# lssfau/ExaStencils

Measured on AMD Instinct MI355X. Metric: LU/s, higher is better.
Workload: dtype f64; 1 GPU; 3D Poisson 7-point Jacobi smoother steps (ghost exchange + sweep + advance), 512 x 512 x 512 cells per GPU, reference field layout (515-double rows); three consecutive steps per pass over HBM (temporal blocking, bit-identical); levels=9, align=0

## Files before the change

### exastencils_amd/csrc/kernels_twostage.hip

```cpp
#include "examg_common.h"

#include <type_traits>

namespace examg {

struct TSGeom {
  int ntx, nty, ntz, zc, nblocks, remap;
  int xs;
  int ys, zs;
  int first;
  Box box1;
  int ax0, ax1, ay0, ay1, az0, az1;
};

constexpr int TS_OUT = 124;

__device__ __forceinline__ long long uniform64(long long v) {
  const unsigned lo = __builtin_amdgcn_readfirstlane((unsigned)v), hi = __builtin_amdgcn_readfirstlane((unsigned)((unsigned long long)v >> 32));
  return (long long)(((unsigned long long)hi << 32) | lo);
}

struct TSProl {
  LayoutDev lc;
  const double *uc;
// ... 498 lines not shown
#undef EXAMG_TS_LAUNCH_ORD
#undef EXAMG_TS_LAUNCH_PF
#undef EXAMG_TS_LAUNCH
  EXAMG_CHECK_LAUNCH("k_two_stage7_lds");
  return 0;
}

template <bool COL>
static int launch_two_stage(const examg_layout_t *lu_, const double *u, const examg_layout_t *lf_, const double *rhs,
                            double *out, const examg_stencil_t *st, double w, int first, const Box &box, hipStream_t s,
                            const Box *box1 = nullptr, const TSProl *prol = nullptr, bool zero_in = false) {
  const Box &b1 = box1 ? *box1 : box;
  int impl = g_ts_lds == -2 ? (box.n1() >= 192 ? 8 : 5) : g_ts_lds;
  if (zero_in && impl == 6) impl = 5;
  if (g_ts_lds == -2 && impl == 8 && !prol && !zero_in && box.count() >= 50000000LL) impl = 83;
  if (impl == 83 && !prol && !zero_in)
    return launch_two_stage_lds<COL, 8, 1, 3>(lu_, u, lf_, rhs, out, st, w, first, box, b1, s, prol, zero_in);
  if (impl == 83) impl = 8;
  if (impl == 8) return launch_two_stage_lds<COL, 8>(lu_, u, lf_, rhs, out, st, w, first, box, b1, s, prol, zero_in);
  if (impl == 6) return launch_two_stage_lds<COL, 6>(lu_, u, lf_, rhs, out, st, w, first, box, b1, s, prol, zero_in);
  return launch_two_stage_lds<COL, 5>(lu_, u, lf_, rhs, out, st, w, first, box, b1, s, prol, zero_in);
}

static bool prolong_args_ok(const char *who, const examg_layout_t *lc, const Box &box) {
  if (box.b0 < 0 || box.b1 < 0 || box.b2 < 0) { set_error("%s: negative fine index", who); return false; }
  int32_t cb[3] = {box.b0 / 2, box.b1 / 2, box.b2 / 2}, ce[3] = {box.e0 / 2 + 1, box.e1 / 2 + 1, box.e2 / 2 + 1};
  if (lc->nd != 3 || !box_inside(lc, make_box(cb, ce), 0)) { set_error("%s: coarse footprint leaves the coarse allocation", who); return false; }
  return true;
}

static bool two_stage_ok(const examg_layout_t *lu, const examg_layout_t *lf, const examg_stencil_t *st, const Box &box) {
  return !g_ts_disable && !lay_split(lu) && !lay_split(lf) && lu->nd == 3 && canonical_order7(st) >= 0 && box.n0() >= 64 && box_inside(lu, box, 1) &&
         box_inside(lf, box, 0);
}

static bool stage_boxes_ok(const examg_layout_t *lf_, const Box &box1, const Box &box2) {
  const LayoutDev lf = make_layout(lf_);
  const bool lo = box1.b0 < box2.b0 && box2.b1 + lf.ref1 == 0 && box2.b2 + lf.ref2 == 0;
  const bool hi = box1.e0 > box2.e0 && box2.e1 + lf.ref1 == lf.tot1 && box2.e2 + lf.ref2 == lf.tot2;
  return !lo && !hi;
}

constexpr int TS3_OUT = 120;

template <int ORDER, int NW, bool NT, int RPW = 3, bool COL = false>
__global__ void __launch_bounds__(64 * NW, 1)
k_three_stage7_lds(LayoutDev lu, const double *__restrict__ u, LayoutDev lf, const double *__restrict__ rhs,
                   double *__restrict__ out, Coef7 k, double w, Box box, TSGeom g) {
  constexpr int NS = RPW * NW;
  constexpr int NO = NS - 4;
  __shared__ d2 SM[3 * 2 * 2 * NW * 64];
#define EB(f, p, h, wq) EBW(wave_rows(wq), f, p, h)
#define EBW(rows, f, p, h) (rows)[((((f) * 2 + (p)) * 2 + (h)) * 64)]
  auto wave_rows = [&](int wq) {
    unsigned off = (unsigned)wq * (3 * 2 * 2 * 64 * 16);
    asm volatile("" : "+s"(off));
    return reinterpret_cast<d2 *>(reinterpret_cast<char *>(SM) + off + threadIdx.x * 16u);
  };
  const int lane = threadIdx.x, wv = __builtin_amdgcn_readfirstlane(threadIdx.y);
  int t = blockIdx.x;
  if (g.remap == 2) {
    const int xy = g.ntx * g.nty;
    const int lz = t / xy, r = t - lz * xy;
    const int per = xy >> 3;
    t = lz * xy + (r < (per << 3) ? (r & 7) * per + (r >> 3) : r);
  }
  const int tx = t % g.ntx;
  t /= g.ntx;
  const int ty = t % g.nty;
  const int tz = t / g.nty;
  const int xw = box.b0 - 4 + TS3_OUT * tx;
  const int xa = xw + 2 * lane;
  const int rw0 = box.b1 + ty * NO;
  const int mb = box.b2 + tz * g.zc;
  const int me = min(mb + g.zc, box.e2);
  const bool inx_a = xa >= box.b0 && xa < box.e0, inx_b = xa + 1 >= box.b0 && xa + 1 < box.e0;
  const bool out_lane = lane >= 2 && lane <= 61;
  const bool st_a = out_lane && inx_a, st_b = out_lane && inx_b;
  const int s0 = RPW * wv;
  int grow[RPW];
  bool row_in[RPW], row_out[RPW];
#pragma unroll
  for (int r = 0; r < RPW; ++r) {
    grow[r] = rw0 - 2 + s0 + r;
    row_in[r] = grow[r] >= box.b1 && grow[r] < box.e1;
    row_out[r] = s0 + r >= 2 && s0 + r <= NS - 3 && row_in[r];
  }
  const bool has_outer = wv == 0 || wv == NW - 1;
  const int outer_row = wv == 0 ? rw0 - 3 : rw0 - 2 + NS;
  const int wlo = wv >= 1 ? wv - 1 : 0, whi = wv + 1 <= NW - 1 ? wv + 1 : NW - 1;

  struct Site {
    const char *row;
    unsigned voff;
  };
  auto site = [&](const double *base, const LayoutDev &l, int R) {
    const int rc = min(max(R + l.ref1, 0), l.tot1 - 1), i0 = xw + l.ref0;
    Site st;
    st.row = reinterpret_cast<const char *>(base + ((long long)i0 + (long long)((unsigned)l.s1 * (unsigned)rc)));
    st.voff = (unsigned)(min(max(2 * lane, -i0 - (rc == 0 ? 0 : 1)), l.tot0 - 1 - i0 - (rc == l.tot1 - 1 ? 1 : 0)) * 8);
    return st;
  };
  struct PlaneCursor {
    int p;
    long long bytes, step;
    int last;
  };
  auto cursor = [&](const LayoutDev &l, int P) {
    PlaneCursor c;
    c.p = P + l.ref2;
    c.last = l.tot2 - 1;
    c.step = uniform64(l.s2 * 8);
    c.bytes = uniform64(l.s2 * 8 * min(max(c.p, 0), c.last));
    return c;
  };
  auto advance = [&](PlaneCursor &c) {
    ++c.p;
    c.bytes += (c.p >= 1 && c.p <= c.last) ? c.step : 0LL;
  };
  auto load_at = [&](const Site &st, long long pb) { return load2(reinterpret_cast<const double *>(st.row + pb + st.voff)); };
  Site urow[RPW], frow[RPW];
#pragma unroll
  for (int r = 0; r < RPW; ++r) {
    urow[r] = site(u, lu, grow[r]);
    frow[r] = site(rhs, lf, grow[r]);
  }
  const Site uouter = site(u, lu, outer_row);
  const int q0 = mb - 2;
  PlaneCursor cu = cursor(lu, q0 - 1), cf = cursor(lf, q0);
  const unsigned vo = (unsigned)lane * 16u;
  char *obase[RPW];
#pragma unroll
  for (int r = 0; r < RPW; ++r)
    obase[r] = reinterpret_cast<char *>(out + ((long long)(xw + lu.ref0) + (long long)((unsigned)lu.s1 * (unsigned)max(grow[r] + lu.ref1, 0))));
  long long obytes = uniform64(lu.s2 * 8 * (long long)(q0 - 2 + lu.ref2));
  const long long ostep = uniform64(lu.s2 * 8);

  d2 U[4][RPW], V[4][RPW], W[4][RPW], F[4][RPW], O[4];
  O[0] = O[1] = O[2] = O[3] = d2{0.0, 0.0};
#pragma unroll
  for (int j = 0; j < 4; ++j) {
#pragma unroll
    for (int r = 0; r < RPW; ++r) U[j][r] = load_at(urow[r], cu.bytes);
    if (has_outer && j >= 1) O[j] = load_at(uouter, cu.bytes);
    advance(cu);
  }
#pragma unroll
  for (int j = 1; j < 3; ++j) {
#pragma unroll
    for (int r = 0; r < RPW; ++r) F[j][r] = load_at(frow[r], cf.bytes);
    advance(cf);
  }
#pragma unroll
  for (int r = 0; r < RPW; ++r) {
    F[0][r] = F[1][r];
    F[3][r] = F[1][r];
#pragma unroll
    for (int j = 0; j < 4; ++j) {
      V[j][r] = U[0][r];
      W[j][r] = U[0][r];
    }
  }
  EB(0, 0, 0, wv) = U[1][0];
  EB(0, 0, 1, wv) = U[1][RPW - 1];
  __builtin_amdgcn_s_waitcnt(0x0F70);
  __syncthreads();

  using I0_ = std::integral_constant<int, 0>;
  using I1_ = std::integral_constant<int, 1>;
  using I2_ = std::integral_constant<int, 2>;
  using I3_ = std::integral_constant<int, 3>;
  auto jac = [&](d2 c, d2 ym, d2 yp, d2 zm, d2 zp, d2 f) {
    const double xl = lane_below0(c.y), xr = lane_above0(c.x);
    const double acc_a = conv7<ORDER>(k, c.x, xl, c.y, ym.x, yp.x, zm.x, zp.x);
    const double acc_b = conv7<ORDER>(k, c.y, c.x, xr, ym.y, yp.y, zm.y, zp.y);
    d2 n;
    n.x = c.x + w * (f.x - acc_a);
    n.y = c.y + w * (f.y - acc_b);
    return n;
  };
  auto jac_x = [&](d2 c, d2 ym, d2 yp, d2 zm, d2 zp, d2 f) {
    const double xl = lane_below0(c.y);
    const double acc = conv7<ORDER>(k, c.x, xl, c.y, ym.x, yp.x, zm.x, zp.x);
    return c.x + w * (f.x - acc);
  };
  auto jac_y = [&](d2 c, d2 ym, d2 yp, d2 zm, d2 zp, d2 f) {
    const double xr = lane_above0(c.x);
    const double acc = conv7<ORDER>(k, c.y, c.x, xr, ym.y, yp.y, zm.y, zp.y);
    return c.y + w * (f.y - acc);
  };
  auto upd = [&](bool first_point, d2 c, d2 ym, d2 yp, d2 zm, d2 zp, d2 f) {
    if constexpr (!COL) return jac(c, ym, yp, zm, zp, f);
    d2 n = c;
    if (first_point) n.x = jac_x(c, ym, yp, zm, zp, f);
    else n.y = jac_y(c, ym, yp, zm, zp, f);
    return n;
  };
  const int cpar = xw + g.first;
  auto step = [&](const int q, auto PHc) {
    constexpr int PH = decltype(PHc)::value;
    d2 (&Um)[RPW] = U[PH & 3], (&Uc)[RPW] = U[(PH + 1) & 3], (&Up)[RPW] = U[(PH + 2) & 3];
    d2 (&Vmm)[RPW] = V[(PH + 3) & 3], (&Vm)[RPW] = V[PH & 3], (&Vn)[RPW] = V[(PH + 1) & 3];
    d2 (&Wmm)[RPW] = W[(PH + 2) & 3], (&Wm)[RPW] = W[(PH + 3) & 3], (&Wn)[RPW] = W[PH & 3];
    d2 (&Fq)[RPW] = F[(PH + 1) & 3], (&Fm)[RPW] = F[PH & 3], (&Fmm)[RPW] = F[(PH + 3) & 3];
    constexpr int ub = PH & 1, vb = (PH + 1) & 1;
    const d2 *const below = wave_rows(wlo), *const above = wave_rows(whi);
    d2 ulo = EBW(below, 0, ub, 1), uhi = EBW(above, 0, ub, 0);
    const d2 vlo = EBW(below, 1, vb, 1), vhi = EBW(above, 1, vb, 0);
    const d2 zlo = EBW(below, 2, vb, 1), zhi = EBW(above, 2, vb, 0);
    if (wv == 0) ulo = O[(PH + 1) & 3];
    if (wv == NW - 1) uhi = O[(PH + 1) & 3];
    const bool pin1 = q >= box.b2 && q < box.e2, pin2 = q - 1 >= box.b2 && q - 1 < box.e2;
    const bool run2 = q >= mb;
    const bool run3 = q - 2 >= mb && q - 2 < me;
    bool fp[RPW];
#pragma unroll
    for (int r = 0; r < RPW; ++r) fp[r] = ((cpar + grow[r] + q) & 1) == 0;
    auto stage1 = [&](auto Rc) {
      constexpr int r = decltype(Rc)::value;
      const d2 c = Uc[r];
      const d2 n = upd(fp[r], c, r == 0 ? ulo : Uc[r == 0 ? 0 : r - 1], r == RPW - 1 ? uhi : Uc[r == RPW - 1 ? r : r + 1], Um[r], Up[r], Fq[r]);
      const bool on = pin1 && row_in[r];
      Vn[r].x = (inx_a && on) ? n.x : c.x;
      Vn[r].y = (inx_b && on) ? n.y : c.y;
    };
    auto stage2 = [&](auto Rc) {
      constexpr int r = decltype(Rc)::value;
      if (run2) {
        const d2 c = Vm[r];
        const d2 n = upd(fp[r], c, r == 0 ? vlo : Vm[r == 0 ? 0 : r - 1], r == RPW - 1 ? vhi : Vm[r == RPW - 1 ? r : r + 1], Vmm[r], Vn[r], Fm[r]);
        const bool on = pin2 && row_in[r];
        Wn[r].x = (inx_a && on) ? n.x : c.x;
        Wn[r].y = (inx_b && on) ? n.y : c.y;
      }
    };
    auto stage3 = [&](auto Rc) {
      constexpr int r = decltype(Rc)::value;
      if (run3 && row_out[r]) {
        const d2 c = Wm[r];
        const d2 o = upd(fp[r], c, r == 0 ? zlo : Wm[r == 0 ? 0 : r - 1], r == RPW - 1 ? zhi : Wm[r == RPW - 1 ? r : r + 1], Wmm[r], Wn[r], Fmm[r]);
        double *qp = reinterpret_cast<double *>(obase[r] + obytes + vo);
        if (st_a && st_b) {
          if (NT) store2_nt(qp, o);
          else store2(qp, o);
        } else if (st_a) {
          qp[0] = o.x;
        } else if (st_b) {
          qp[1] = o.y;
        }
      }
    };
    if constexpr (RPW == 3) {
      stage1(I1_{});
      stage2(I1_{});
      stage3(I1_{});
      stage1(I0_{});
      stage1(I2_{});
      stage2(I0_{});
      stage2(I2_{});
      stage3(I0_{});
      stage3(I2_{});
    } else {
      stage1(I0_{});
      stage1(I1_{});
      stage2(I0_{});
      stage2(I1_{});
      stage3(I0_{});
      stage3(I1_{});
    }
    if (q <= me) {
      d2 *const own = wave_rows(wv);
      EBW(own, 0, vb, 0) = Up[0];
      EBW(own, 0, vb, 1) = Up[RPW - 1];
      EBW(own, 1, ub, 0) = Vn[0];
      EBW(own, 1, ub, 1) = Vn[RPW - 1];
      EBW(own, 2, ub, 0) = Wn[0];
      EBW(own, 2, ub, 1) = Wn[RPW - 1];
    }
#pragma unroll
    for (int r = 0; r < RPW; ++r) {
      Um[r] = load_at(urow[r], cu.bytes);
      Fmm[r] = load_at(frow[r], cf.bytes);
    }
    if (has_outer) O[PH & 3] = load_at(uouter, cu.bytes);
    advance(cu);
    advance(cf);
    obytes += ostep;
    __syncthreads();
#ifndef TS3_NO_SCHED_BARRIER
    __builtin_amdgcn_sched_barrier(0);
#endif
  };
  const int qe = me + 1;
  for (int q = q0; q <= qe; q += 4) {
    step(q, I0_{});
    step(q + 1, I1_{});
    step(q + 2, I2_{});
    step(q + 3, I3_{});
  }
#undef EB
#undef EBW
}

static thread_local int g_ts3_zc = -1;
static thread_local int g_ts3_disable = 0;
static thread_local long long g_ts3_minpts = 8000000LL;

static bool three_stage_ok(const examg_layout_t *lu, const examg_layout_t *lf, const examg_stencil_t *st, const Box &box) {
  if (g_ts3_disable || !two_stage_ok(lu, lf, st, box) || box.n1() < 20 || box.count() < g_ts3_minpts) return false;
  const LayoutDev u = make_layout(lu), f = make_layout(lf);
  return u.s2 < (1LL << 32) && f.s2 < (1LL << 32);
}

template <int NW, int RPW, bool COL>
static int launch_three_stage_shape(const examg_layout_t *lu_, const double *u, const examg_layout_t *lf_, const double *rhs, double *out,
                                    const examg_stencil_t *st, double w, const Box &box, hipStream_t s, int first) {
  constexpr int NO = RPW * NW - 4;
  const LayoutDev lu = make_layout(lu_), lf = make_layout(lf_);
  TSGeom g;
  g.xs = g.ys = g.zs = 0;
  g.ntx = (box.n0() + TS3_OUT - 1) / TS3_OUT;
  g.nty = (box.n1() + NO - 1) / NO;
  const int xy = g.ntx * g.nty, n2 = box.n2();
  int zc = n2;
  {
    long long best = -1;
    for (int t = 1; t <= (n2 + 7) / 8; ++t) {
      const int c = (n2 + t - 1) / t, tt = (n2 + c - 1) / c;
      if ((c > 64 && t < (n2 + 7) / 8) || (c < 16 && t > 1)) continue;
      const long long cost = (((long long)xy * tt + 255) / 256) * (((c + 4 + 3) & ~3) + 4);
      if (best < 0 || cost < best) { best = cost; zc = c; }
    }
    if (zc + 3 < n2) zc = (zc + 3) & ~3;
  }
  if (g_ts3_zc > 0) zc = g_ts3_zc;
  if (zc > n2) zc = n2;
  g.zc = zc;
  g.ntz = (n2 + zc - 1) / zc;
  g.nblocks = xy * g.ntz;
  g.remap = g_ts_remap >= 0 ? g_ts_remap : 2;
  g.first = first;
  g.box1 = box;
  g.ax0 = -lu.ref0; g.ax1 = lu.tot0 - lu.ref0;
  g.ay0 = -lu.ref1; g.ay1 = lu.tot1 - lu.ref1;
  g.az0 = -lu.ref2; g.az1 = lu.tot2 - lu.ref2;
  Coef7 k;
  for (int i = 0; i < 7; ++i) k.c[i] = st->coef[i];
  const int ord = canonical_order7(st);
  const bool nt = g_ts_nt >= 0 ? g_ts_nt != 0 : box.count() * 24LL > 200000000LL;
  dim3 block(64, NW, 1), grid(g.nblocks, 1, 1);
#define EXAMG_TS3(ORD, NTV) hipLaunchKernelGGL((k_three_stage7_lds<ORD, NW, NTV, RPW, COL>), grid, block, 0, s, lu, u, lf, rhs, out, k, w, box, g)
  if (ord == 0) {
    if (nt) EXAMG_TS3(0, true);
    else EXAMG_TS3(0, false);
  } else {
    if (nt) EXAMG_TS3(1, true);
    else EXAMG_TS3(1, false);
  }
#undef EXAMG_TS3
  EXAMG_CHECK_LAUNCH("k_three_stage7_lds");
  return 0;
}

static int launch_three_stage(const examg_layout_t *lu, const double *u, const examg_layout_t *lf, const double *rhs, double *out,
                              const examg_stencil_t *st, double w, const Box &box, hipStream_t s) {
  return launch_three_stage_shape<8, 3, false>(lu, u, lf, rhs, out, st, w, box, s, 0);
}

static int launch_three_colours(const examg_layout_t *lu, const double *u, const examg_layout_t *lf, const double *rhs, double *out,
                                const examg_stencil_t *st, double w, int first, const Box &box, hipStream_t s) {
  return launch_three_stage_shape<8, 3, true>(lu, u, lf, rhs, out, st, w, box, s, first);
}

}

using namespace examg;

#ifdef EXAMG_DEBUG_HOOKS
extern "C" int examg_debug_two_stage_lds(int nw) {
  g_ts_lds = nw < 0 ? -2 : nw;
  return 0;
}

extern "C" int examg_debug_two_stage_nt(int nt) {
  g_ts_nt = nt < 0 ? -1 : (nt ? 1 : 0);
  return 0;
}

extern "C" int examg_debug_two_stage_prol(int wpe) {
  if (wpe >= 10) g_ts_wpe = wpe - 10 == 4 ? 4 : 1;
  else g_ts_prol_wpe = wpe == 1 ? 1 : 4;
  return 0;
}

extern "C" int examg_debug_three_stage(int disable, int zc) {
  g_ts3_disable = disable == 1;
  g_ts3_minpts = disable == 2 ? (1LL << 20) : 8000000LL;
  g_ts3_zc = zc > 0 ? zc : -1;
  return 0;
}

extern "C" int examg_debug_two_stage(int disable, int blocks, int remap, int wy) {
  g_ts_disable = disable;
  if (blocks != 0) g_ts_blocks = blocks > 0 ? blocks : -1;
  if (remap >= 0) g_ts_remap = remap;
  g_ts_minzc = wy > 0 ? wy : -1;
  return 0;
}
#endif

extern "C" int examg_two_stage_eligible(const examg_layout_t *lu, const examg_layout_t *lf, const examg_stencil_t *st,
                                        const int32_t *begin1, const int32_t *end1, const int32_t *begin2, const int32_t *end2) {
  if (!lu || !lf || !st || !begin1 || !end1 || !begin2 || !end2) return 0;
  const Box box1 = make_box(begin1, end1), box2 = make_box(begin2, end2);
  if (box2.count() == 0) return 0;
  if (box2.b0 < box1.b0 || box2.b1 < box1.b1 || box2.b2 < box1.b2 || box2.e0 > box1.e0 || box2.e1 > box1.e1 || box2.e2 > box1.e2) return 0;
  if (box1.b0 == box2.b0 && box1.b1 == box2.b1 && box1.b2 == box2.b2 && box1.e0 == box2.e0 && box1.e1 == box2.e1 && box1.e2 == box2.e2 &&
      small_two_stage_ok(lu, lf, st, box2))
    return 1;
  if (!(two_stage_ok(lu, lf, st, box2) && box_inside(lu, box1, 1) && box_inside(lf, box1, 0) && stage_boxes_ok(lf, box1, box2))) return 0;
  const LayoutDev u = make_layout(lu), f = make_layout(lf);
  return (u.s2 < (1LL << 32) && f.s2 < (1LL << 32)) ? 1 : 0;
}

extern "C" int examg_rbgs_sweep_fused(const examg_layout_t *lu, const double *u_in, double *u_out,
                                      const examg_layout_t *lf, const double *rhs, const examg_stencil_t *st, double w,
                                      int first, const int32_t *begin, const int32_t *end, examg_stream_t stream) {
  if (!lu || !u_in || !u_out || !lf || !rhs || !st || !begin || !end) { set_error("examg_rbgs_sweep_fused: null argument"); return 1; }
  if (u_in == u_out) { set_error("examg_rbgs_sweep_fused: out of place only"); return 1; }
  if (first != 0 && first != 1) { set_error("examg_rbgs_sweep_fused: first colour must be 0 or 1"); return 1; }
  const Box box = make_box(begin, end);
  if (box.count() == 0) return 0;
  if (two_stage_ok(lu, lf, st, box)) return launch_two_stage<true>(lu, u_in, lf, rhs, u_out, st, w, first, box, (hipStream_t)stream);
  if (small_two_stage_ok(lu, lf, st, box)) return launch_small_two_stage(true, 0, lu, u_in, u_out, lf, rhs, st, w, first, box, nullptr, nullptr, (hipStream_t)stream);
  const int reach = stencil_reach(st);
  int32_t b2[3], e2[3];
  for (int d = 0; d < 3; ++d) {
    const bool on = d < lu->nd;
    b2[d] = begin[d] - (on ? reach : 0);
    e2[d] = end[d] + (on ? reach : 0);
  }
  int rc = examg_axpby(lu, u_in, lu, u_out, 1.0, 0.0, b2, e2, stream);
  if (rc) return rc;
  rc = examg_rbgs_colour(lu, u_out, lf, rhs, st, w, first, begin, end, stream);
  if (rc) return rc;
  return examg_rbgs_colour(lu, u_out, lf, rhs, st, w, 1 - first, begin, end, stream);
}

extern "C" int examg_rbgs_sweep_fused_zero(const examg_layout_t *lu, double *u_out, const examg_layout_t *lf, const double *rhs,
                                           const examg_stencil_t *st, double w, int first, const int32_t *begin,
                                           const int32_t *end, examg_stream_t stream) {
  if (!lu || !u_out || !lf || !rhs || !st || !begin || !end) { set_error("examg_rbgs_sweep_fused_zero: null argument"); return 1; }
  if (first != 0 && first != 1) { set_error("examg_rbgs_sweep_fused_zero: first colour must be 0 or 1"); return 1; }
  const Box box = make_box(begin, end);
  if (box.count() == 0) return 0;
  if (two_stage_ok(lu, lf, st, box))
    return launch_two_stage<true>(lu, u_out, lf, rhs, u_out, st, w, first, box, (hipStream_t)stream, nullptr, nullptr, true);
  if (small_two_stage_ok(lu, lf, st, box)) return launch_small_two_stage(true, 2, lu, nullptr, u_out, lf, rhs, st, w, first, box, nullptr, nullptr, (hipStream_t)stream);
  const int reach = stencil_reach(st);
  int32_t b2[3], e2[3];
  for (int d = 0; d < 3; ++d) {
    const bool on = d < lu->nd;
    b2[d] = begin[d] - (on ? reach : 0);
    e2[d] = end[d] + (on ? reach : 0);
  }
  int rc = examg_set(lu, u_out, 0.0, b2, e2, stream);
  if (rc) return rc;
  rc = examg_rbgs_colour(lu, u_out, lf, rhs, st, w, first, begin, end, stream);
  if (rc) return rc;
  return examg_rbgs_colour(lu, u_out, lf, rhs, st, w, 1 - first, begin, end, stream);
}

extern "C" int examg_rbgs_sweep_fused_prolong(const examg_layout_t *lu, const double *u_in, double *u_out,
                                              const examg_layout_t *lf, const double *rhs, const examg_stencil_t *st, double w,
                                              int first, const int32_t *begin, const int32_t *end, const examg_layout_t *lc,
                                              const double *uc, examg_stream_t stream) {
  if (!lu || !u_in || !u_out || !lf || !rhs || !st || !begin || !end || !lc || !uc) { set_error("examg_rbgs_sweep_fused_prolong: null argument"); return 1; }
  if (u_in == u_out) { set_error("examg_rbgs_sweep_fused_prolong: out of place only"); return 1; }
  if (first != 0 && first != 1) { set_error("examg_rbgs_sweep_fused_prolong: first colour must be 0 or 1"); return 1; }
  const Box box = make_box(begin, end);
  if (box.count() == 0) return 0;
  if (two_stage_ok(lu, lf, st, box)) {
    if (!prolong_args_ok("examg_rbgs_sweep_fused_prolong", lc, box)) return 1;
    TSProl pr;
    pr.lc = make_layout(lc);
    pr.uc = uc;
    return launch_two_stage<true>(lu, u_in, lf, rhs, u_out, st, w, first, box, (hipStream_t)stream, nullptr, &pr);
  }
  if (small_two_stage_ok(lu, lf, st, box)) {
    if (!prolong_args_ok("examg_rbgs_sweep_fused_prolong", lc, box)) return 1;
    return launch_small_two_stage(true, 1, lu, u_in, u_out, lf, rhs, st, w, first, box, lc, uc, (hipStream_t)stream);
  }
  const int reach = stencil_reach(st);
  int32_t b2[3], e2[3];
  for (int d = 0; d < 3; ++d) {
    const bool on = d < lu->nd;
    b2[d] = begin[d] - (on ? reach : 0);
    e2[d] = end[d] + (on ? reach : 0);
  }
  int rc = examg_axpby(lu, u_in, lu, u_out, 1.0, 0.0, b2, e2, stream);
  if (rc) return rc;
  rc = examg_prolong_add(lc, uc, lu, u_out, begin, end, stream);
  if (rc) return rc;
  rc = examg_rbgs_colour(lu, u_out, lf, rhs, st, w, first, begin, end, stream);
  if (rc) return rc;
  return examg_rbgs_colour(lu, u_out, lf, rhs, st, w, 1 - first, begin, end, stream);
}

extern "C" int examg_rbgs_sweep_fused_boxes(const examg_layout_t *lu, const double *u_in, double *u_out, double *tmp,
                                            const examg_layout_t *lf, const double *rhs, const examg_stencil_t *st, double w,
                                            int first, const int32_t *begin1, const int32_t *end1, const int32_t *begin2,
                                            const int32_t *end2, examg_stream_t stream) {
  if (!lu || !u_in || !u_out || !lf || !rhs || !st || !begin1 || !end1 || !begin2 || !end2) { set_error("examg_rbgs_sweep_fused_boxes: null argument"); return 1; }
  if (u_in == u_out) { set_error("examg_rbgs_sweep_fused_boxes: out of place only"); return 1; }
  if (first != 0 && first != 1) { set_error("examg_rbgs_sweep_fused_boxes: first colour must be 0 or 1"); return 1; }
  const Box box1 = make_box(begin1, end1), box2 = make_box(begin2, end2);
  if (box2.count() == 0) return 0;
  if (box2.b0 < box1.b0 || box2.b1 < box1.b1 || box2.b2 < box1.b2 || box2.e0 > box1.e0 || box2.e1 > box1.e1 || box2.e2 > box1.e2) {
    set_error("examg_rbgs_sweep_fused_boxes: the second box must lie inside the first");
    return 1;
  }
  if (two_stage_ok(lu, lf, st, box2) && box_inside(lu, box1, 1) && box_inside(lf, box1, 0) && stage_boxes_ok(lf, box1, box2))
    return launch_two_stage<true>(lu, u_in, lf, rhs, u_out, st, w, first, box2, (hipStream_t)stream, &box1);
  if (box1.b0 == box2.b0 && box1.b1 == box2.b1 && box1.b2 == box2.b2 && box1.e0 == box2.e0 && box1.e1 == box2.e1 && box1.e2 == box2.e2 &&
      small_two_stage_ok(lu, lf, st, box2))
    return launch_small_two_stage(true, 0, lu, u_in, u_out, lf, rhs, st, w, first, box2, nullptr, nullptr, (hipStream_t)stream);
  if (!tmp || tmp == u_in || tmp == u_out) { set_error("examg_rbgs_sweep_fused_boxes: fallback needs a distinct tmp array"); return 1; }
  const int reach = stencil_reach(st);
  int32_t b2[3], e2[3];
  for (int d = 0; d < 3; ++d) {
    const bool on = d < lu->nd;
    b2[d] = begin1[d] - (on ? reach : 0);
    e2[d] = end1[d] + (on ? reach : 0);
  }
  int rc = examg_axpby(lu, u_in, lu, tmp, 1.0, 0.0, b2, e2, stream);
  if (rc) return rc;
  rc = examg_rbgs_colour(lu, tmp, lf, rhs, st, w, first, begin1, end1, stream);
  if (rc) return rc;
  rc = examg_axpby(lu, tmp, lu, u_out, 1.0, 0.0, begin2, end2, stream);
  if (rc) return rc;
  return examg_stencil_op(EXAMG_SMOOTH, lu, tmp, lf, rhs, lu, u_out, st, w, 1 - first, begin2, end2, stream);
}

extern "C" int examg_jacobi2_boxes(const examg_layout_t *lu, const double *u_in, double *u_out, double *tmp,
                                   const examg_layout_t *lf, const double *rhs, const examg_stencil_t *st, double w,
                                   const int32_t *begin1, const int32_t *end1, const int32_t *begin2, const int32_t *end2,
                                   examg_stream_t stream) {
  if (!lu || !u_in || !u_out || !lf || !rhs || !st || !begin1 || !end1 || !begin2 || !end2) { set_error("examg_jacobi2_boxes: null argument"); return 1; }
  if (u_in == u_out) { set_error("examg_jacobi2_boxes: out of place only"); return 1; }
  const Box box1 = make_box(begin1, end1), box2 = make_box(begin2, end2);
  if (box2.count() == 0) return 0;
  if (box2.b0 < box1.b0 || box2.b1 < box1.b1 || box2.b2 < box1.b2 || box2.e0 > box1.e0 || box2.e1 > box1.e1 || box2.e2 > box1.e2) {
    set_error("examg_jacobi2_boxes: the stage-2 box must lie inside the stage-1 box");
    return 1;
  }
  if (two_stage_ok(lu, lf, st, box2) && box_inside(lu, box1, 1) && box_inside(lf, box1, 0) && stage_boxes_ok(lf, box1, box2))
    return launch_two_stage<false>(lu, u_in, lf, rhs, u_out, st, w, 0, box2, (hipStream_t)stream, &box1);
  if (box1.b0 == box2.b0 && box1.b1 == box2.b1 && box1.b2 == box2.b2 && box1.e0 == box2.e0 && box1.e1 == box2.e1 && box1.e2 == box2.e2 &&
      small_two_stage_ok(lu, lf, st, box2))
    return launch_small_two_stage(false, 0, lu, u_in, u_out, lf, rhs, st, w, 0, box2, nullptr, nullptr, (hipStream_t)stream);
  if (const int r27 = sf27_jacobi2_try(lu, u_in, u_out, lf, rhs, st, w, box1, box2, (hipStream_t)stream)) return r27 < 0 ? 1 : 0;
  if (!tmp || tmp == u_in || tmp == u_out) { set_error("examg_jacobi2_boxes: fallback needs a distinct tmp array"); return 1; }
  const int reach = stencil_reach(st);
  int32_t b2[3], e2[3];
  for (int d = 0; d < 3; ++d) {
    const bool on = d < lu->nd;
    b2[d] = begin1[d] - (on ? reach : 0);
    e2[d] = end1[d] + (on ? reach : 0);
  }
  int rc = examg_axpby(lu, u_in, lu, tmp, 1.0, 0.0, b2, e2, stream);
  if (rc) return rc;
  rc = examg_jacobi(lu, u_in, tmp, lf, rhs, st, w, begin1, end1, stream);
  if (rc) return rc;
  return examg_jacobi(lu, tmp, u_out, lf, rhs, st, w, begin2, end2, stream);
}

extern "C" int examg_jacobi2_prolong(const examg_layout_t *lu, const double *u_in, double *u_out, double *tmp,
                                     const examg_layout_t *lf, const double *rhs, const examg_stencil_t *st, double w,
                                     const int32_t *begin, const int32_t *end, const examg_layout_t *lc, const double *uc,
                                     examg_stream_t stream) {
  if (!lu || !u_in || !u_out || !lf || !rhs || !st || !begin || !end || !lc || !uc) { set_error("examg_jacobi2_prolong: null argument"); return 1; }
  if (u_in == u_out) { set_error("examg_jacobi2_prolong: out of place only"); return 1; }
  const Box box = make_box(begin, end);
  if (box.count() == 0) return 0;
  if (two_stage_ok(lu, lf, st, box)) {
    if (!prolong_args_ok("examg_jacobi2_prolong", lc, box)) return 1;
    TSProl pr;
    pr.lc = make_layout(lc);
    pr.uc = uc;
    return launch_two_stage<false>(lu, u_in, lf, rhs, u_out, st, w, 0, box, (hipStream_t)stream, nullptr, &pr);
  }
  if (small_two_stage_ok(lu, lf, st, box)) {
    if (!prolong_args_ok("examg_jacobi2_prolong", lc, box)) return 1;
    return launch_small_two_stage(false, 1, lu, u_in, u_out, lf, rhs, st, w, 0, box, lc, uc, (hipStream_t)stream);
  }
  if (!tmp || tmp == u_in || tmp == u_out) { set_error("examg_jacobi2_prolong: fallback needs a distinct tmp array"); return 1; }
  const int reach = stencil_reach(st);
  int32_t b2[3], e2[3];
  for (int d = 0; d < 3; ++d) {
    const bool on = d < lu->nd;
    b2[d] = begin[d] - (on ? reach : 0);
    e2[d] = end[d] + (on ? reach : 0);
  }
  int rc = examg_axpby(lu, u_in, lu, u_out, 1.0, 0.0, b2, e2, stream);
  if (rc) return rc;
  rc = examg_axpby(lu, u_in, lu, tmp, 1.0, 0.0, b2, e2, stream);
  if (rc) return rc;
  rc = examg_prolong_add(lc, uc, lu, u_out, begin, end, stream);
  if (rc) return rc;
  rc = examg_jacobi(lu, u_out, tmp, lf, rhs, st, w, begin, end, stream);
  if (rc) return rc;
  return examg_jacobi(lu, tmp, u_out, lf, rhs, st, w, begin, end, stream);
}

extern "C" int examg_jacobi2(const examg_layout_t *lu, const double *u_in, double *u_out, double *tmp,
                             const examg_layout_t *lf, const double *rhs, const examg_stencil_t *st, double w,
                             const int32_t *begin, const int32_t *end, examg_stream_t stream) {
  if (!lu || !u_in || !u_out || !lf || !rhs || !st || !begin || !end) { set_error("examg_jacobi2: null argument"); return 1; }
  if (u_in == u_out) { set_error("examg_jacobi2: out of place only"); return 1; }
  const Box box = make_box(begin, end);
  if (box.count() == 0) return 0;
  if (two_stage_ok(lu, lf, st, box)) return launch_two_stage<false>(lu, u_in, lf, rhs, u_out, st, w, 0, box, (hipStream_t)stream);
  if (small_two_stage_ok(lu, lf, st, box)) return launch_small_two_stage(false, 0, lu, u_in, u_out, lf, rhs, st, w, 0, box, nullptr, nullptr, (hipStream_t)stream);
  if (const int r27 = sf27_jacobi2_try(lu, u_in, u_out, lf, rhs, st, w, box, box, (hipStream_t)stream)) return r27 < 0 ? 1 : 0;
  if (!tmp || tmp == u_in || tmp == u_out) { set_error("examg_jacobi2: fallback needs a distinct tmp array"); return 1; }
  const int reach = stencil_reach(st);
  int32_t b2[3], e2[3];
  for (int d = 0; d < 3; ++d) {
    const bool on = d < lu->nd;
    b2[d] = begin[d] - (on ? reach : 0);
    e2[d] = end[d] + (on ? reach : 0);
  }
  int rc = examg_axpby(lu, u_in, lu, tmp, 1.0, 0.0, b2, e2, stream);
  if (rc) return rc;
  rc = examg_jacobi(lu, u_in, tmp, lf, rhs, st, w, begin, end, stream);
  if (rc) return rc;
  return examg_jacobi(lu, tmp, u_out, lf, rhs, st, w, begin, end, stream);
}

extern "C" int examg_jacobi3(const examg_layout_t *lu, const double *u_in, double *u_out, double *tmp, const examg_layout_t *lf,
                             const double *rhs, const examg_stencil_t *st, double w, const int32_t *begin, const int32_t *end,
                             examg_stream_t stream) {
  if (!lu || !u_in || !u_out || !lf || !rhs || !st || !begin || !end) { set_error("examg_jacobi3: null argument"); return 1; }
  if (u_in == u_out) { set_error("examg_jacobi3: out of place only"); return 1; }
  const Box box = make_box(begin, end);
  if (box.count() == 0) return 0;
  if (three_stage_ok(lu, lf, st, box)) return launch_three_stage(lu, u_in, lf, rhs, u_out, st, w, box, (hipStream_t)stream);
  if (!tmp || tmp == u_in || tmp == u_out) { set_error("examg_jacobi3: fallback needs a distinct tmp array"); return 1; }
  const int reach = stencil_reach(st);
  int32_t b2[3], e2[3];
  for (int d = 0; d < 3; ++d) {
    const bool on = d < lu->nd;
    b2[d] = begin[d] - (on ? reach : 0);
    e2[d] = end[d] + (on ? reach : 0);
  }
  int rc = examg_axpby(lu, u_in, lu, tmp, 1.0, 0.0, b2, e2, stream);
  if (rc) return rc;
  rc = examg_jacobi(lu, u_in, tmp, lf, rhs, st, w, begin, end, stream);
  if (rc) return rc;
  if (examg_two_stage_eligible(lu, lf, st, begin, end, begin, end))
    return examg_jacobi2(lu, tmp, u_out, nullptr, lf, rhs, st, w, begin, end, stream);
  rc = examg_axpby(lu, u_in, lu, u_out, 1.0, 0.0, b2, e2, stream);
  if (rc) return rc;
  rc = examg_jacobi(lu, tmp, u_out, lf, rhs, st, w, begin, end, stream);
  if (rc) return rc;
  rc = examg_jacobi(lu, u_out, tmp, lf, rhs, st, w, begin, end, stream);
  if (rc) return rc;
  return examg_axpby(lu, tmp, lu, u_out, 1.0, 0.0, begin, end, stream);
}

extern "C" int examg_three_stage_eligible(const examg_layout_t *lu, const examg_layout_t *lf, const examg_stencil_t *st, const int32_t *begin,
                                          const int32_t *end) {
  if (!lu || !lf || !st || !begin || !end) return 0;
  return three_stage_ok(lu, lf, st, make_box(begin, end)) ? 1 : 0;
}

extern "C" int examg_rbgs_colours3(const examg_layout_t *lu, const double *u_in, double *u_out, const examg_layout_t *lf, const double *rhs,
                                   const examg_stencil_t *st, double w, int first, const int32_t *begin, const int32_t *end,
                                   examg_stream_t stream) {
  if (!lu || !u_in || !u_out || !lf || !rhs || !st || !begin || !end) { set_error("examg_rbgs_colours3: null argument"); return 1; }
  if (u_in == u_out) { set_error("examg_rbgs_colours3: out of place only"); return 1; }
  if (first != 0 && first != 1) { set_error("examg_rbgs_colours3: first colour must be 0 or 1"); return 1; }
  const Box box = make_box(begin, end);
  if (box.count() == 0) return 0;
  if (three_stage_ok(lu, lf, st, box)) return launch_three_colours(lu, u_in, lf, rhs, u_out, st, w, first, box, (hipStream_t)stream);
  const int reach = stencil_reach(st);
  int32_t b2[3], e2[3];
  for (int d = 0; d < 3; ++d) {
    const bool on = d < lu->nd;
    b2[d] = begin[d] - (on ? reach : 0);
    e2[d] = end[d] + (on ? reach : 0);
  }
  int rc = examg_axpby(lu, u_in, lu, u_out, 1.0, 0.0, b2, e2, stream);
  for (int k = 0; k < 3 && !rc; ++k) rc = examg_rbgs_colour(lu, u_out, lf, rhs, st, w, (k & 1) ? 1 - first : first, begin, end, stream);
  return rc;
}
```

Before: 588.0 billion LU/s.

## Add point-per-lane three-stage kernel shape with cost-model selection

Adds a three-stage temporally blocked Jacobi kernel variant where each lane handles one x point and each wave holds six rows, giving taller y tiles with less halo overlap. A cost model weighs block counts and z-chunk length for the old pair-shape and the new point-shape and picks the cheaper one per box. The new layout trades x-direction halo waste (58 of 64 lanes output) for reduced y-redundancy and more register rows per thread, which may increase register pressure.

```diff
diff --git a/exastencils_amd/csrc/kernels_twostage.hip b/exastencils_amd/csrc/kernels_twostage.hip
--- a/exastencils_amd/csrc/kernels_twostage.hip
+++ b/exastencils_amd/csrc/kernels_twostage.hip
@@ -824,7 +824,242 @@
 #undef EBW
 }
 
+constexpr int TS3P_OUT = 58;
+
+template <int ORDER, int NW, bool NT, int RPW = 6>
+__global__ void __launch_bounds__(64 * NW, 1)
+k_three_stage7_lds_pt(LayoutDev lu, const double *__restrict__ u, LayoutDev lf, const double *__restrict__ rhs,
+                      double *__restrict__ out, Coef7 k, double w, Box box, TSGeom g) {
+  constexpr int NS = RPW * NW;
+  constexpr int NO = NS - 4;
+  __shared__ double SM[3 * 2 * 2 * NW * 64];
+#define EBW(rows, f, p, h) (rows)[((((f) * 2 + (p)) * 2 + (h)) * 64)]
+  auto wave_rows = [&](int wq) {
+    unsigned off = (unsigned)wq * (3 * 2 * 2 * 64 * 8);
+    asm volatile("" : "+s"(off));
+    return reinterpret_cast<double *>(reinterpret_cast<char *>(SM) + off + threadIdx.x * 8u);
+  };
+  const int lane = threadIdx.x, wv = __builtin_amdgcn_readfirstlane(threadIdx.y);
+  int t = blockIdx.x;
+  if (g.remap == 2) {
+    const int xy = g.ntx * g.nty;
+    const int lz = t / xy, r = t - lz * xy;
+    const int per = xy >> 3;
+    t = lz * xy + (r < (per << 3) ? (r & 7) * per + (r >> 3) : r);
+  }
+  const int tx = t % g.ntx;
+  t /= g.ntx;
+  const int ty = t % g.nty;
+  const int tz = t / g.nty;
+  const int xw = box.b0 - 3 + TS3P_OUT * tx;
+  const int xa = xw + lane;
+  const int rw0 = box.b1 + ty * NO;
+  const int mb = box.b2 + tz * g.zc;
+  const int me = min(mb + g.zc, box.e2);
+  const bool inx = xa >= box.b0 && xa < box.e0;
+  const bool st = lane >= 3 && lane <= 60 && inx;
+  const int s0 = RPW * wv;
+  const int grow0 = rw0 - 2 + s0;
+  unsigned rin = 0, rout = 0;
+#pragma unroll
+  for (int r = 0; r < RPW; ++r) {
+    const bool in = grow0 + r >= box.b1 && grow0 + r < box.e1;
+    rin |= (in ? 1u : 0u) << r;
+    rout |= ((in && s0 + r >= 2 && s0 + r <= NS - 3) ? 1u : 0u) << r;
+  }
+  rin = __builtin_amdgcn_readfirstlane(rin);
+  rout = __builtin_amdgcn_readfirstlane(rout);
+  const bool has_outer = wv == 0 || wv == NW - 1;
+  const int outer_row = wv == 0 ? rw0 - 3 : rw0 - 2 + NS;
+  const int wlo = wv >= 1 ? wv - 1 : 0, whi = wv + 1 <= NW - 1 ? wv + 1 : NW - 1;
+
+  typedef const __attribute__((address_space(1))) double *gcptr;
+  typedef __attribute__((address_space(1))) double *gptr;
+  auto rowclamp = [&](const LayoutDev &l, int R) { return min(max(R + l.ref1, 0), l.tot1 - 1); };
+  auto rowbase = [&](const double *base, const LayoutDev &l, int R) {
+    return reinterpret_cast<long long>(base + ((long long)(xw + l.ref0) + (long long)((unsigned)l.s1 * (unsigned)rowclamp(l, R))));
+  };
+  auto laneoff = [&](const LayoutDev &l) {
+    const int i0 = xw + l.ref0;
+    return (unsigned)(min(max(lane, -i0), l.tot0 - 1 - i0) * 8);
+  };
+  auto pin = [&](long long b) {
+    asm("" : "+s"(b));
+    return b;
+  };
+  auto ld = [&](long long b, unsigned &voff) {
+    asm volatile("" : "+v"(voff));
+    return *reinterpret_cast<gcptr>(b + voff);
+  };
+  unsigned uoff[RPW], foff[RPW], uoff_outer = laneoff(lu);
+#pragma unroll
+  for (int r = 0; r < RPW; ++r) {
+    uoff[r] = laneoff(lu) + (unsigned)(rowclamp(lu, grow0 + r) - rowclamp(lu, grow0)) * ((unsigned)lu.s1 * 8u);
+    foff[r] = laneoff(lf) + (unsigned)(rowclamp(lf, grow0 + r) - rowclamp(lf, grow0)) * ((unsigned)lf.s1 * 8u);
+  }
+  const long long ubase = rowbase(u, lu, grow0), fbase = rowbase(rhs, lf, grow0), uouter = rowbase(u, lu, outer_row);
+  auto load_rows = [&](double (&dst)[RPW], long long b, unsigned (&voff)[RPW]) {
+    b = pin(b);
+#pragma unroll
+    for (int r = 0; r < RPW; ++r) dst[r] = ld(b, voff[r]);
+  };
+  struct PlaneCursor {
+    int p;
+    long long bytes, step;
+    int last;
+  };
+  auto cursor = [&](const LayoutDev &l, int P) {
+    PlaneCursor c;
+    c.p = P + l.ref2;
+    c.last = l.tot2 - 1;
+    c.step = uniform64(l.s2 * 8);
+    c.bytes = uniform64(l.s2 * 8 * min(max(c.p, 0), c.last));
+    return c;
+  };
+  auto advance = [&](PlaneCursor &c) {
+    ++c.p;
+    c.bytes += (c.p >= 1 && c.p <= c.last) ? c.step : 0LL;
+  };
+  const int q0 = mb - 2;
+  PlaneCursor cu = cursor(lu, q0 - 1), cf = cursor(lf, q0);
+  long long optr = uniform64(rowbase(out, lu, grow0) + 8 * lu.s2 * (long long)(q0 - 2 + lu.ref2));
+
+  double U[4][RPW], V[4][RPW], W[4][RPW], F[4][RPW], O[4];
+  O[0] = O[1] = O[2] = O[3] = 0.0;
+#pragma unroll
+  for (int j = 0; j < 4; ++j) {
+    load_rows(U[j], ubase + cu.bytes, uoff);
+    if (has_outer && j >= 1) O[j] = ld(pin(uouter + cu.bytes), uoff_outer);
+    advance(cu);
+  }
+#pragma unroll
+  for (int j = 1; j < 3; ++j) {
+    load_rows(F[j], fbase + cf.bytes, foff);
+    advance(cf);
+  }
+#pragma unroll
+  for (int r = 0; r < RPW; ++r) {
+    F[0][r] = F[1][r];
+    F[3][r] = F[1][r];
+#pragma unroll
+    for (int j = 0; j < 4; ++j) {
+      V[j][r] = U[0][r];
+      W[j][r] = U[0][r];
+    }
+  }
+  {
+    double *const own = wave_rows(wv);
+    EBW(own, 0, 0, 0) = U[1][0];
+    EBW(own, 0, 0, 1) = U[1][RPW - 1];
+  }
+  __builtin_amdgcn_s_waitcnt(0x0F70);
+  __syncthreads();
+
+  using I0_ = std::integral_constant<int, 0>;
+  using I1_ = std::integral_constant<int, 1>;
+  using I2_ = std::integral_constant<int, 2>;
+  using I3_ = std::integral_constant<int, 3>;
+  using IL_ = std::integral_constant<int, RPW - 1>;
+  auto jac = [&](double c, double ym, double yp, double zm, double zp, double f) {
+    const double xl = lane_below0(c), xr = lane_above0(c);
+    const double acc = conv7<ORDER>(k, c, xl, xr, ym, yp, zm, zp);
+    return c + w * (f - acc);
+  };
+  auto sel = [&](bool on, double a, double b) {
+    const int lo = on ? __double2loint(a) : __double2loint(b), hi = on ? __double2hiint(a) : __double2hiint(b);
+    return __hiloint2double(hi, lo);
+  };
+  auto step = [&](const int q, auto PHc) {
+    constexpr int PH = decltype(PHc)::value;
+    double (&Um)[RPW] = U[PH & 3], (&Uc)[RPW] = U[(PH + 1) & 3], (&Up)[RPW] = U[(PH + 2) & 3];
+    double (&Vmm)[RPW] = V[(PH + 3) & 3], (&Vm)[RPW] = V[PH & 3], (&Vn)[RPW] = V[(PH + 1) & 3];
+    double (&Wmm)[RPW] = W[(PH + 2) & 3], (&Wm)[RPW] = W[(PH + 3) & 3], (&Wn)[RPW] = W[PH & 3];
+    double (&Fq)[RPW] = F[(PH + 1) & 3], (&Fm)[RPW] = F[PH & 3], (&Fmm)[RPW] = F[(PH + 3) & 3];
+    constexpr int ub = PH & 1, vb = (PH + 1) & 1;
+    asm volatile("" : "+s"(rin));
+    asm volatile("" : "+s"(rout));
+    asm volatile("" : "+s"(optr));
+    const double *const below = wave_rows(wlo), *const above = wave_rows(whi);
+    double ulo = EBW(below, 0, ub, 1), uhi = EBW(above, 0, ub, 0);
+    const double vlo = EBW(below, 1, vb, 1), vhi = EBW(above, 1, vb, 0);
+    const double zlo = EBW(below, 2, vb, 1), zhi = EBW(above, 2, vb, 0);
+    if (wv == 0) ulo = O[(PH + 1) & 3];
+    if (wv == NW - 1) uhi = O[(PH + 1) & 3];
+    const unsigned rin1 = (q >= box.b2 && q < box.e2) ? rin : 0u, rin2 = (q - 1 >= box.b2 && q - 1 < box.e2) ? rin : 0u;
+    const bool run2 = q >= mb;
+    const bool run3 = q - 2 >= mb && q - 2 < me;
+    auto stage1 = [&](auto Rc) {
+      constexpr int r = decltype(Rc)::value;
+      const double c = Uc[r];
+      const double n = jac(c, r == 0 ? ulo : Uc[r == 0 ? 0 : r - 1], r == RPW - 1 ? uhi : Uc[r == RPW - 1 ? r : r + 1], Um[r], Up[r], Fq[r]);
+      Vn[r] = sel(inx && ((rin1 >> r) & 1u), n, c);
+    };
+    auto stage2 = [&](auto Rc) {
+      constexpr int r = decltype(Rc)::value;
+      if (run2) {
+        const double c = Vm[r];
+        const double n = jac(c, r == 0 ? vlo : Vm[r == 0 ? 0 : r - 1], r == RPW - 1 ? vhi : Vm[r == RPW - 1 ? r : r + 1], Vmm[r], Vn[r], Fm[r]);
+        Wn[r] = sel(inx && ((rin2 >> r) & 1u), n, c);
+      }
+    };
+    auto stage3 = [&](auto Rc) {
+      constexpr int r = decltype(Rc)::value;
+      if (run3 && ((rout >> r) & 1u)) {
+        const double c = Wm[r];
+        const double o = jac(c, r == 0 ? zlo : Wm[r == 0 ? 0 : r - 1], r == RPW - 1 ? zhi : Wm[r == RPW - 1 ? r : r + 1], Wmm[r], Wn[r], Fmm[r]);
+        if (st) {
+          asm volatile("" : "+v"(uoff[r]));
+          const gptr qp = reinterpret_cast<gptr>(optr + uoff[r]);
+          if (NT) __builtin_nontemporal_store(o, qp);
+          else *qp = o;
+        }
+      }
+    };
+    auto rows = [&](auto Rc) {
+      stage1(Rc);
+      stage2(Rc);
+      stage3(Rc);
+    };
+    if constexpr (RPW >= 3) rows(I1_{});
+    if constexpr (RPW >= 4) rows(I2_{});
+    if constexpr (RPW >= 5) rows(I3_{});
+    if constexpr (RPW >= 6) rows(std::integral_constant<int, 4>{});
+    stage1(I0_{});
+    stage1(IL_{});
+    stage2(I0_{});
+    stage2(IL_{});
+    stage3(I0_{});
+    stage3(IL_{});
+    if (q <= me) {
+      double *const own = wave_rows(wv);
+      EBW(own, 0, vb, 0) = Up[0];
+      EBW(own, 0, vb, 1) = Up[RPW - 1];
+      EBW(own, 1, ub, 0) = Vn[0];
+      EBW(own, 1, ub, 1) = Vn[RPW - 1];
+      EBW(own, 2, ub, 0) = Wn[0];
+      EBW(own, 2, ub, 1) = Wn[RPW - 1];
+    }
+    load_rows(Um, ubase + cu.bytes, uoff);
+    load_rows(Fmm, fbase + cf.bytes, foff);
+    if (has_outer) O[PH & 3] = ld(pin(uouter + cu.bytes), uoff_outer);
+    advance(cu);
+    advance(cf);
+    optr += cu.step;
+    __syncthreads();
+    __builtin_amdgcn_sched_barrier(0);
+  };
+  const int qe = me + 1;
+  for (int q = q0; q <= qe; q += 4) {
+    step(q, I0_{});
+    step(q + 1, I1_{});
+    step(q + 2, I2_{});
+    step(q + 3, I3_{});
+  }
+#undef EBW
+}
+
 static thread_local int g_ts3_zc = -1;
+static thread_local int g_ts3_shape = -1;
 static thread_local int g_ts3_disable = 0;
 static thread_local long long g_ts3_minpts = 8000000LL;
 
@@ -834,32 +1069,56 @@
   return u.s2 < (1LL << 32) && f.s2 < (1LL << 32);
 }
 
-template <int NW, int RPW, bool COL>
-static int launch_three_stage_shape(const examg_layout_t *lu_, const double *u, const examg_layout_t *lf_, const double *rhs, double *out,
-                                    const examg_stencil_t *st, double w, const Box &box, hipStream_t s, int first) {
-  constexpr int NO = RPW * NW - 4;
+struct TS3Plan {
+  int shape, ntx, nty, ntz, zc;
+  long long cost;
+};
+constexpr int TS3_W_PAIR = 1493, TS3_W_POINT = 1900;
+constexpr int TS3_ZC_CAP_PAIR = 64, TS3_ZC_CAP_POINT = 64;
+
+static TS3Plan three_stage_plan(int shape, const Box &box) {
+  TS3Plan p;
+  p.shape = shape;
+  const int xout = shape == 1 ? TS3P_OUT : TS3_OUT, yout = shape == 1 ? 6 * 8 - 4 : 3 * 8 - 4;
+  const int cap = shape == 1 ? TS3_ZC_CAP_POINT : TS3_ZC_CAP_PAIR;
+  p.ntx = (box.n0() + xout - 1) / xout;
+  p.nty = (box.n1() + yout - 1) / yout;
+  const int xy = p.ntx * p.nty, n2 = box.n2();
+  int zc = n2;
+  long long best = -1;
+  for (int t = 1; t <= (n2 + 7) / 8; ++t) {
+    const int c = (n2 + t - 1) / t, tt = (n2 + c - 1) / c;
+    if ((c > cap && t < (n2 + 7) / 8) || (c < 16 && t > 1)) continue;
+    const long long cost = (((long long)xy * tt + 255) / 256) * (((c + 4 + 3) & ~3) + 4);
+    if (best < 0 || cost < best) { best = cost; zc = c; }
+  }
+  if (zc + 3 < n2) zc = (zc + 3) & ~3;
+  if (g_ts3_zc > 0) zc = g_ts3_zc;
+  if (zc > n2) zc = n2;
+  p.zc = zc;
+  p.ntz = (n2 + zc - 1) / zc;
+  p.cost = (((long long)xy * p.ntz + 255) / 256) * (((zc + 4 + 3) & ~3) + 4) * (shape == 1 ? TS3_W_POINT : TS3_W_PAIR);
+  return p;
+}
+
+static TS3Plan three_stage_choose(const examg_layout_t *lu, const examg_layout_t *lf, const Box &box) {
+  const bool point_ok = make_layout(lu).s1 * 48 < (1LL << 32) && make_layout(lf).s1 * 48 < (1LL << 32);
+  if (g_ts3_shape >= 0) return three_stage_plan(point_ok ? g_ts3_shape : 0, box);
+  const TS3Plan a = three_stage_plan(0, box), b = three_stage_plan(1, box);
+  return point_ok && b.cost < a.cost ? b : a;
+}
+
+template <int NW, bool COL>
+static int launch_three_stage_shape(const TS3Plan &p, const examg_layout_t *lu_, const double *u, const examg_layout_t *lf_, const double *rhs,
+                                    double *out, const examg_stencil_t *st, double w, const Box &box, hipStream_t s, int first) {
   const LayoutDev lu = make_layout(lu_), lf = make_layout(lf_);
   TSGeom g;
   g.xs = g.ys = g.zs = 0;
-  g.ntx = (box.n0() + TS3_OUT - 1) / TS3_OUT;
-  g.nty = (box.n1() + NO - 1) / NO;
-  const int xy = g.ntx * g.nty, n2 = box.n2();
-  int zc = n2;
-  {
-    long long best = -1;
-    for (int t = 1; t <= (n2 + 7) / 8; ++t) {
-      const int c = (n2 + t - 1) / t, tt = (n2 + c - 1) / c;
-      if ((c > 64 && t < (n2 + 7) / 8) || (c < 16 && t > 1)) continue;
-      const long long cost = (((long long)xy * tt + 255) / 256) * (((c + 4 + 3) & ~3) + 4);
-      if (best < 0 || cost < best) { best = cost; zc = c; }
-    }
-    if (zc + 3 < n2) zc = (zc + 3) & ~3;
-  }
-  if (g_ts3_zc > 0) zc = g_ts3_zc;
-  if (zc > n2) zc = n2;
-  g.zc = zc;
-  g.ntz = (n2 + zc - 1) / zc;
-  g.nblocks = xy * g.ntz;
+  g.ntx = p.ntx;
+  g.nty = p.nty;
+  g.zc = p.zc;
+  g.ntz = p.ntz;
+  g.nblocks = p.ntx * p.nty * p.ntz;
   g.remap = g_ts_remap >= 0 ? g_ts_remap : 2;
   g.first = first;
   g.box1 = box;
@@ -871,7 +1130,15 @@
   const int ord = canonical_order7(st);
   const bool nt = g_ts_nt >= 0 ? g_ts_nt != 0 : box.count() * 24LL > 200000000LL;
   dim3 block(64, NW, 1), grid(g.nblocks, 1, 1);
-#define EXAMG_TS3(ORD, NTV) hipLaunchKernelGGL((k_three_stage7_lds<ORD, NW, NTV, RPW, COL>), grid, block, 0, s, lu, u, lf, rhs, out, k, w, box, g)
+#define EXAMG_TS3(ORD, NTV)                                                                                                             \
+  do {                                                                                                                                  \
+    if constexpr (!COL) {                                                                                                               \
+      if (p.shape == 1) hipLaunchKernelGGL((k_three_stage7_lds_pt<ORD, NW, NTV, 6>), grid, block, 0, s, lu, u, lf, rhs, out, k, w, box, g); \
+      else hipLaunchKernelGGL((k_three_stage7_lds<ORD, NW, NTV, 3, false>), grid, block, 0, s, lu, u, lf, rhs, out, k, w, box, g);      \
+    } else {                                                                                                                            \
+      hipLaunchKernelGGL((k_three_stage7_lds<ORD, NW, NTV, 3, true>), grid, block, 0, s, lu, u, lf, rhs, out, k, w, box, g);            \
+    }                                                                                                                                   \
+  } while (0)
   if (ord == 0) {
     if (nt) EXAMG_TS3(0, true);
     else EXAMG_TS3(0, false);
@@ -886,12 +1153,12 @@
 
 static int launch_three_stage(const examg_layout_t *lu, const double *u, const examg_layout_t *lf, const double *rhs, double *out,
                               const examg_stencil_t *st, double w, const Box &box, hipStream_t s) {
-  return launch_three_stage_shape<8, 3, false>(lu, u, lf, rhs, out, st, w, box, s, 0);
+  return launch_three_stage_shape<8, false>(three_stage_choose(lu, lf, box), lu, u, lf, rhs, out, st, w, box, s, 0);
 }
 
 static int launch_three_colours(const examg_layout_t *lu, const double *u, const examg_layout_t *lf, const double *rhs, double *out,
                                 const examg_stencil_t *st, double w, int first, const Box &box, hipStream_t s) {
-  return launch_three_stage_shape<8, 3, true>(lu, u, lf, rhs, out, st, w, box, s, first);
+  return launch_three_stage_shape<8, true>(three_stage_plan(0, box), lu, u, lf, rhs, out, st, w, box, s, first);
 }
 
 }
@@ -919,6 +1186,20 @@
   g_ts3_disable = disable == 1;
   g_ts3_minpts = disable == 2 ? (1LL << 20) : 8000000LL;
   g_ts3_zc = zc > 0 ? zc : -1;
+  return 0;
+}
+
+extern "C" int examg_debug_three_stage_shape(int shape) {
+  g_ts3_shape = (shape == 0 || shape == 1) ? shape : -1;
+  return 0;
+}
+
+extern "C" int examg_debug_three_stage_plan(const examg_layout_t *lu, const examg_layout_t *lf, const int32_t *begin, const int32_t *end, int *out) {
+  if (!lu || !lf || !begin || !end || !out) return 1;
+  const Box box = make_box(begin, end);
+  if (box.count() == 0 || lu->nd != 3) return 1;
+  const TS3Plan p = three_stage_choose(lu, lf, box);
+  out[0] = p.shape; out[1] = p.ntx; out[2] = p.nty; out[3] = p.ntz; out[4] = p.zc;
   return 0;
 }
 
```

Result: slower. 571.8 billion LU/s (-2.8%).
